# LordLiang/DrawingSpinUp

Hardware: AMD Instinct MI355X
Metric: drawings/sec end-to-end (512x512, 6 views, 24 frames) (higher is better)
Workload: dtype f16 (diffusion) / f16 table + f32 MLP (NSR) / f32 (stage-1 deformable convolutions, IS-Net, contour) / f32 with bf16 x 3 products (stage-2 convolutions; the reference: cuDNN TF32)

## Files before the change

### drawingspinup_amd/csrc/hashgrid_mfma.hip

```cpp
#include "hashgrid_dev.h"
#include "partial_reduce.h"
#include "tr_stage.h"

#include <type_traits>

using namespace dsu_hg;

namespace {

typedef float f32x16 __attribute__((ext_vector_type(16)));
typedef __bf16 bf16x8 __attribute__((ext_vector_type(8)));

__device__ __forceinline__ void softplus_inplace2(f32x16& acc, int r) {
  const f32x2 h = softplus100_pair(f32x2{acc[r], acc[r + 1]});
  acc[r] = h.x;
  acc[r + 1] = h.y;
}

__device__ __forceinline__ void bf16_split8(const float* x, bf16x8& hi, bf16x8& mid) {
#pragma unroll
  for (int i = 0; i < 8; ++i) {
    const __bf16 h = (__bf16)x[i];
    hi[i] = h;
    mid[i] = (__bf16)(x[i] - (float)h);
// ... 961 lines not shown
      const float dga = ax == 0 ? dg[0] : (ax == 1 ? dg[1] : dg[2]);
      dout0 = valid ? sgn * 0.5f * dga / eps + dl / eps2 : 0.0f;
    };
    if (e < 7) {
#pragma unroll
      for (int l = 0; l < ACT; ++l) vm_take(rw[l]);
      prep_unpack();
      prep_point(e);
      prep_request(e);
      prep_dout(e);
    }
#pragma unroll 1
    for (; e < 7; e += e_step) {
      gb1[0] += dout0;
      const float other0 = partner32(dout0, h);
      const float d0h0 = h == 0 ? dout0 : other0;
      const float d0h1 = h == 1 ? dout0 : other0;
      bf16x8 obh0, obm0, obh1, obm1;
      if constexpr (L0BF)
        pack_operands(in, std::integral_constant<int, (2 * KPA <= 16 ? 2 * KPA : 16)>{}, obh0, obm0, obh1, obm1);
#pragma unroll
      for (int half = 0; half < 2; ++half) {
        if (half == 1 && !live1) break;
        weights_per_use();
        const float d0 = half ? d0h1 : d0h0;
        f32x16 Hh[2];
        if constexpr (L0BF) l0_bf(half ? obh1 : obh0, half ? obm1 : obm0, Hh);
        else l0_half(in, half, Hh);
        softplus2(Hh);
#pragma unroll
        for (int T = 0; T < 2; ++T)
#pragma unroll
          for (int r = 0; r < 16; ++r) gw1c0[T][r] = fmaf(Hh[T][r], d0, gw1c0[T][r]);
        f32x16 din;
#pragma unroll
        for (int r = 0; r < 16; ++r) din[r] = 0.0f;
#pragma unroll
        for (int T = 0; T < 2; ++T) {
          float dpre[16];
#pragma unroll
          for (int q = 0; q < 4; ++q) {
            const float4 w = *reinterpret_cast<const float4*>(&lds[wo + PW_W1O0 + 32 * T + 8 * q + 4 * h]);
            dpre[4 * q + 0] = w.x * d0;
            dpre[4 * q + 1] = w.y * d0;
            dpre[4 * q + 2] = w.z * d0;
            dpre[4 * q + 3] = w.w * d0;
          }
          din_tile(T, dpre, Hh[T], din);
        }
        if (h == half) stage_in_T(in);
        __builtin_amdgcn_wave_barrier();
        gemm_T(gw0);
        __builtin_amdgcn_wave_barrier();
        store_din(e, din, wave_first + half * 32 + l31, r1);
      }
      const int en = e + e_step < 7 ? e + e_step : 6;
      handover();
      prep_unpack();
      prep_point(en);
      prep_request(en);
      prep_dout(en);
    }
#pragma unroll
    for (int T = 0; T < 2; ++T)
#pragma unroll
      for (int r = 0; r < 16; ++r) {
        float c0 = gw1c0[T][r];
#pragma unroll
        for (int off = 16; off > 0; off >>= 1) c0 += __shfl_xor(c0, off);
        if (l31 == gw1_col(0)) gw0[T][r] += c0;
      }
  }

  __syncthreads();
  float* red = lds;
  {
    float* rr = red + wave * PART_STRIDE;
#pragma unroll
    for (int T = 0; T < 2; ++T)
#pragma unroll
      for (int r = 0; r < 16; ++r) {
        const int feat = feat_of(T, r, h);
        const bool input = l31 < 2 * ACT || (l31 >= 2 * NL && l31 < 2 * NL + 4);
        rr[PART_GW0 + feat * 32 + l31] = input ? gw0[T][r] : 0.0f;
        const int o = l31 >= 2 * NL + 4 ? l31 - (2 * NL + 4) : (l31 >= 2 * ACT && l31 < 2 * ACT + NOUT - 8 ? l31 - 2 * ACT + 8 : -1);
        if (o >= 0) rr[PART_GW1 + feat * 32 + o] = gw0[T][r];
        if (l31 >= NOUT) rr[PART_GW1 + feat * 32 + l31] = 0.0f;
      }
#pragma unroll
    for (int o = 0; o < NOUT; ++o) gb1[o] += __shfl_xor(gb1[o], 32);
#pragma unroll
    for (int off = 16; off > 0; off >>= 1)
#pragma unroll
      for (int o = 0; o < NOUT; ++o) gb1[o] += __shfl_xor(gb1[o], off);
    if (lane == 0) {
#pragma unroll
      for (int o = 0; o < NOUT; ++o) rr[PART_GB1 + o] = gb1[o];
    }
  }
  __syncthreads();
  float* part = partials + (size_t)blockIdx.x * PART_STRIDE;
  for (int v = threadIdx.x; v < PART_GB1 + NOUT; v += blockDim.x)
    part[v] = (red[v] + red[PART_STRIDE + v]) + (red[2 * PART_STRIDE + v] + red[3 * PART_STRIDE + v]);
}

template <int NL, int ACT>
bool launch_bwd_pipe_one(uint32_t active, int blocks, hipStream_t s, const dsu_sdf_mlp& mlp,
                         const float* pts, int64_t n, float radius, float eps, float eps2,
                         const float* d_sdf, const float* d_grad, const float* d_feature,
                         const float* d_laplace, float* partials, const __half2* enc, float2* dinbuf,
                         const int32_t* perm) {
  if ((int)active != ACT) return false;
  sdf_fd_bwd_pipe_kernel<NL, ACT><<<dim3(blocks), dim3(256), 0, s>>>(
      mlp, pts, n, radius, eps, eps2, d_sdf, d_grad, d_feature, d_laplace, partials, enc, dinbuf, perm);
  return true;
}

template <int NL>
bool launch_bwd_pipe(uint32_t active, int blocks, hipStream_t s, const dsu_sdf_mlp& mlp,
                     const float* pts, int64_t n, float radius, float eps, float eps2,
                     const float* d_sdf, const float* d_grad, const float* d_feature,
                     const float* d_laplace, float* partials, const __half2* enc, float2* dinbuf,
                     const int32_t* perm) {
#define DSU_PIPE_TRY(A)                                                                          \
  if (launch_bwd_pipe_one<NL, A>(active, blocks, s, mlp, pts, n, radius, eps, eps2, d_sdf,       \
                                 d_grad, d_feature, d_laplace, partials, enc, dinbuf, perm))      \
    return true;
  DSU_PIPE_TRY(4) DSU_PIPE_TRY(5) DSU_PIPE_TRY(6) DSU_PIPE_TRY(7)
#undef DSU_PIPE_TRY
  return false;
}

constexpr int SC_MAXBLOCKS = 768;
constexpr int SC_THREADS = 256;
constexpr int SC_QCAP = 512;
constexpr int SC_LOG2 = 10;
constexpr int SC_SLOTS = 1 << SC_LOG2;
constexpr int SC_LDS_F = SC_SLOTS + 4 * SC_SLOTS + (SC_THREADS / 64) * 3 * SC_QCAP;
constexpr int SC_TILE_CAP = (SC_LDS_F * 4) / 16;
constexpr int SC_BBOX_OFF = SC_LDS_F;
constexpr int SC_LDS_TOTAL = SC_LDS_F + 16;
static_assert(SC_QCAP % 4 == 0 && SC_QCAP >= 512, "queue: one full evaluation of a wave must fit");

__device__ __forceinline__ uint32_t sc_slot(uint32_t entry) {
  return (entry * 2654435761u) >> (32 - SC_LOG2);
}
__device__ __forceinline__ void sc_commit_from(uint32_t* keys, unsigned long long* acc,
                                               float* __restrict__ gtable, uint32_t entry,
                                               uint32_t slot, float v0, float v1) {
#pragma unroll
  for (int probe = 1; probe < 3; ++probe) {
    slot = (slot + 1) & (SC_SLOTS - 1);
    const uint32_t old = atomicCAS(&keys[slot], GC_EMPTY, entry);
    if (old == GC_EMPTY || old == entry) {
      atomicAdd(&acc[2 * slot], gc_fix(v0));
      atomicAdd(&acc[2 * slot + 1], gc_fix(v1));
      return;
    }
  }
  unsafeAtomicAdd(gtable + (size_t)entry * 2, v0);
  unsafeAtomicAdd(gtable + (size_t)entry * 2 + 1, v1);
}

struct OwnReduce {
  const float* partials;
  int nblocks;
  float *g_w0, *g_b0, *g_w1, *g_b1;
};
constexpr int OWN_RED_BLOCKS = (PART_GB1 + NOUT + 63) / 64;

template <int NL>
__device__ __forceinline__ void reduce_own_block(const OwnReduce& o, int blk, float* red) {
  const int e = threadIdx.x & 63, g = threadIdx.x >> 6, ng = blockDim.x >> 6;
  const int v = blk * 64 + e;
  const bool in_range = v < PART_GB1 + NOUT;
  for (int sl = g; sl < 16; sl += ng) {
    float acc = 0.0f;
    if (in_range)
      for (int b = sl; b < o.nblocks; b += 16) acc += o.partials[(size_t)b * PART_STRIDE + v];
    red[sl * 64 + e] = acc;
  }
  __syncthreads();
  if (g != 0 || !in_range) return;
  float s = 0.0f;
#pragma unroll
  for (int k = 0; k < 16; ++k) s += red[k * 64 + e];
  if (v < PART_GW1) {
    const int feat = v >> 5, k = v & 31;
    if (k < MC<NL>::KIN) {
      const int c = ref_col<NL>(k);
      if (c >= 0) o.g_w0[feat * MC<NL>::DIN + c] += s;
      else o.g_b0[feat] += s;
    }
  } else if (v < PART_GB1) {
    const int feat = (v - PART_GW1) >> 5, oo = (v - PART_GW1) & 31;
    if (oo < NOUT) o.g_w1[oo * HID + feat] += s;
  } else {
    o.g_b1[v - PART_GB1] += s;
  }
}

template <int NL>
__global__ __launch_bounds__(SC_THREADS) void sdf_fd_scatter_kernel(
    GridMeta m, const float* __restrict__ pts, int64_t n, float radius, float eps, uint32_t active,
    const float2* __restrict__ dinbuf, float* __restrict__ gtable, int merge_levels,
    int centre_acc, int dense_levels, int* __restrict__ work_counter, OwnReduce own,
    dsu_partial_reduce extra) {
  extern __shared__ __attribute__((aligned(16))) float lds[];
  const int n_red_own = own.partials ? OWN_RED_BLOCKS : 0;
  const int n_red = n_red_own + (extra.partials ? dsu_red::blocks_of(extra) : 0);
  if ((int)blockIdx.x < n_red) {
    if ((int)blockIdx.x < n_red_own) reduce_own_block<NL>(own, blockIdx.x, lds);
    else dsu_red::reduce_block(extra, blockIdx.x - n_red_own, lds);
    return;
  }
  const int sc_block = (int)blockIdx.x - n_red, sc_grid = (int)gridDim.x - n_red;
  uint32_t* c_keys = reinterpret_cast<uint32_t*>(lds);
  unsigned long long* c_acc = reinterpret_cast<unsigned long long*>(lds + SC_SLOTS);
  const int lane = threadIdx.x & 63, wave = threadIdx.x >> 6;
  float* qbase = lds + 5 * SC_SLOTS + wave * 3 * SC_QCAP;
  uint32_t* q_ent = reinterpret_cast<uint32_t*>(qbase);
  float* q_v0 = qbase + SC_QCAP;
  float* q_v1 = qbase + 2 * SC_QCAP;
  unsigned long long* tile = reinterpret_cast<unsigned long long*>(lds);
  int* bbox = reinterpret_cast<int*>(lds + SC_BBOX_OFF);
  for (int t = threadIdx.x; t < SC_SLOTS; t += blockDim.x) {
    c_keys[t] = GC_EMPTY;
    c_acc[2 * t] = 0ull;
    c_acc[2 * t + 1] = 0ull;
  }
  if (threadIdx.x < 12) bbox[threadIdx.x] = (threadIdx.x % 6) < 3 ? 0x7fffffff : -0x7fffffff;
  int region = 0;
  __syncthreads();
  const int64_t n_chunks = (n + blockDim.x - 1) / blockDim.x;
  const int64_t n_items = n_chunks * (int64_t)active;
  int* next_slot = reinterpret_cast<int*>(lds + SC_BBOX_OFF) + 12;
  int64_t cur = sc_block, nxt = (int64_t)sc_block + sc_grid;
  float pn[3] = {0.f, 0.f, 0.f};
  float2 dnx[7];
#pragma unroll
  for (int e = 0; e < 7; ++e) dnx[e] = make_float2(0.f, 0.f);
  auto request = [&](int64_t item) {
    const int64_t chunk = item / (int64_t)active;
    const uint32_t lv = (uint32_t)(item - chunk * (int64_t)active);
    int64_t idx = chunk * blockDim.x + threadIdx.x;
    idx = idx < n ? idx : n - 1;
    pn[0] = pts[idx * 3]; pn[1] = pts[idx * 3 + 1]; pn[2] = pts[idx * 3 + 2];
#pragma unroll
    for (int e = 0; e < 7; ++e) dnx[e] = dinbuf[((size_t)e * active + lv) * n + idx];
  };
  if (cur < n_items) request(cur);
  int parity = 0;
  int qn = 0;
  auto drain = [&]() {
    __builtin_amdgcn_wave_barrier();
    for (int i0 = 0; i0 < qn; i0 += 64) {
      const int qi = i0 + lane;
      if (qi < qn) {
        const uint32_t ent = q_ent[qi];
        const float a0 = q_v0[qi], a1 = q_v1[qi];
        const uint32_t slot = sc_slot(ent);
        const uint32_t old = atomicCAS(&c_keys[slot], GC_EMPTY, ent);
        if (old == GC_EMPTY || old == ent) {
          atomicAdd(&c_acc[2 * slot], gc_fix(a0));
          atomicAdd(&c_acc[2 * slot + 1], gc_fix(a1));
        } else {
          sc_commit_from(c_keys, c_acc, gtable, ent, slot, a0, a1);
        }
      }
    }
    __builtin_amdgcn_wave_barrier();
    qn = 0;
  };
  auto flush_cache = [&]() {
    for (int t = threadIdx.x; t < SC_SLOTS; t += blockDim.x) {
      const uint32_t key = c_keys[t];
      if (key != GC_EMPTY) {
        unsafeAtomicAdd(gtable + (size_t)key * 2, gc_unfix(c_acc[2 * t]));
        unsafeAtomicAdd(gtable + (size_t)key * 2 + 1, gc_unfix(c_acc[2 * t + 1]));
        c_keys[t] = GC_EMPTY;
        c_acc[2 * t] = 0ull;
        c_acc[2 * t + 1] = 0ull;
      }
    }
  };

#pragma unroll 1
  while (cur < n_items) {
    {
      const int64_t chunk = cur / (int64_t)active;
      const int lev = (int)(cur - chunk * (int64_t)active);
      const float l_scale = m.scale[lev];
      const uint32_t l_off = m.off[lev], hsize = m.off[lev + 1] - m.off[lev];
      const uint32_t l_res = m.res[lev], l_hashed = m.hashed[lev];
      const int64_t i = chunk * blockDim.x + threadIdx.x;
      const bool valid = i < n;
      const float p[3] = {pn[0], pn[1], pn[2]};
      float2 dv[7];
#pragma unroll
      for (int e = 0; e < 7; ++e) {
        dv[e].x = valid ? dnx[e].x : 0.0f;
        dv[e].y = valid ? dnx[e].y : 0.0f;
      }
      if (nxt < n_items) request(nxt);
      if (threadIdx.x == 0) *next_slot = 2 * sc_grid + atomicAdd(work_counter, 1);
      const CellPos ccp = cell_of(l_scale, contract(p[0], radius), contract(p[1], radius),
                                  contract(p[2], radius));
      float2 D0 = dv[0], Da[3];
      uint32_t left = 0u;
      const bool inside = fabsf(p[0]) <= radius && fabsf(p[1]) <= radius && fabsf(p[2]) <= radius;
      int lo[3], hi[3];
#pragma unroll
      for (int a = 0; a < 3; ++a) {
        Da[a] = make_float2(0.f, 0.f);
        lo[a] = valid ? (int)ccp.c[a] : 0x7fffffff;
        hi[a] = valid ? (int)ccp.c[a] : -0x7fffffff;
      }
#pragma unroll
      for (int e = 1; e < 7; ++e) {
        const int ax = (e - 1) >> 1;
        const float off = ((e - 1) & 1) ? -eps : eps;
        const float qa = fminf(fmaxf(p[ax] + off, -radius), radius);
        const float posa = fmaf(l_scale, contract(qa, radius), 0.5f);
        const float fl = floorf(posa);
        const bool same = ((uint32_t)(int)fl == ccp.c[ax]) & (centre_acc != 0) & inside;
        const float delta = posa - ((float)(int)ccp.c[ax] + ccp.f[ax]);
        D0.x += same ? dv[e].x : 0.0f;
        D0.y += same ? dv[e].y : 0.0f;
        Da[ax].x += same ? dv[e].x * delta : 0.0f;
        Da[ax].y += same ? dv[e].y * delta : 0.0f;
        left |= (valid & !same) ? (1u << e) : 0u;
        if (valid & inside) {
          lo[ax] = min(lo[ax], (int)fl);
          hi[ax] = max(hi[ax], (int)fl);
        }
      }
      if (valid & !inside) {
#pragma unroll 1
        for (int e = 1; e < 7; ++e) {
          float q[3];
          fd_point(p, e, eps, radius, q);
          const CellPos cq = cell_of(l_scale, contract(q[0], radius), contract(q[1], radius),
                                     contract(q[2], radius));
#pragma unroll
          for (int a = 0; a < 3; ++a) {
            lo[a] = min(lo[a], (int)cq.c[a]);
            hi[a] = max(hi[a], (int)cq.c[a]);
          }
        }
      }
      bool dense = false;
      int x0 = 0, y0 = 0, z0 = 0, ddx = 1, ddxy = 1, vol = 0;
      int64_t after_next;
      {
        int* bb = bbox + 6 * parity;
#pragma unroll
        for (int a = 0; a < 3; ++a) {
#pragma unroll
          for (int off = 32; off > 0; off >>= 1) {
            lo[a] = min(lo[a], __shfl_xor(lo[a], off));
            hi[a] = max(hi[a], __shfl_xor(hi[a], off));
          }
        }
        if (lane == 0) {
#pragma unroll
          for (int a = 0; a < 3; ++a) {
            atomicMin(&bb[a], lo[a]);
            atomicMax(&bb[3 + a], hi[a]);
          }
        }
        __syncthreads();
        after_next = *next_slot;
        x0 = bb[0]; y0 = bb[1]; z0 = bb[2];
        const long long ex = (long long)bb[3] - x0 + 2, ey = (long long)bb[4] - y0 + 2,
                        ez = (long long)bb[5] - z0 + 2;
        if (dense_levels && bb[3] >= bb[0] && ex * ey * ez <= (long long)SC_TILE_CAP && ex < 4096 && ey < 4096) {
          dense = true;
          ddx = (int)ex; ddxy = (int)(ex * ey); vol = (int)(ex * ey * ez);
        }
        if (threadIdx.x < 6) bbox[6 * (parity ^ 1) + threadIdx.x] = threadIdx.x < 3 ? 0x7fffffff : -0x7fffffff;
        parity ^= 1;
      }
      if ((int)dense != region) {
        if (region == 0) {
          for (int t = threadIdx.x; t < SC_TILE_CAP * 2; t += blockDim.x) tile[t] = 0ull;
        } else {
          for (int t = threadIdx.x; t < SC_SLOTS; t += blockDim.x) {
            c_keys[t] = GC_EMPTY;
            c_acc[2 * t] = 0ull;
            c_acc[2 * t + 1] = 0ull;
          }
        }
        region = (int)dense;
        __syncthreads();
      }

#pragma unroll 1
      for (int e = 1; e < 8; ++e) {
        CellPos cp = ccp;
        float v[16];
        bool flush;
        if (e < 7) {
          flush = (left >> e) & 1u;
          if (__ballot(flush) == 0ull) continue;
          float2 d = dv[1];
#pragma unroll
          for (int k = 2; k < 7; ++k) {
            d.x = e == k ? dv[k].x : d.x;
            d.y = e == k ? dv[k].y : d.y;
          }
          float q[3];
          fd_point(p, e, eps, radius, q);
          cp = cell_of(l_scale, contract(q[0], radius), contract(q[1], radius), contract(q[2], radius));
#pragma unroll
          for (int c = 0; c < 8; ++c) {
            const float w = corner_weight(cp, c);
            v[2 * c] = w * d.x;
            v[2 * c + 1] = w * d.y;
          }
        } else {
          const float X[2] = {1.0f - cp.f[0], cp.f[0]}, Y[2] = {1.0f - cp.f[1], cp.f[1]},
                      Z[2] = {1.0f - cp.f[2], cp.f[2]};
#pragma unroll
          for (int c = 0; c < 8; ++c) {
            const int cx_ = c & 1, cy_ = (c >> 1) & 1, cz_ = (c >> 2) & 1;
            const float yz = Y[cy_] * Z[cz_], xz = X[cx_] * Z[cz_], xy = X[cx_] * Y[cy_];
            const float w = X[cx_] * yz;
            const float gx = cx_ ? yz : -yz, gy = cy_ ? xz : -xz, gz = cz_ ? xy : -xy;
            v[2 * c] = fmaf(D0.x, w, fmaf(Da[0].x, gx, fmaf(Da[1].x, gy, Da[2].x * gz)));
            v[2 * c + 1] = fmaf(D0.y, w, fmaf(Da[0].y, gx, fmaf(Da[1].y, gy, Da[2].y * gz)));
          }
          flush = valid;
        }
        const int key = flush ? (int)((cp.c[0] & 1023u) | ((cp.c[1] & 1023u) << 10) | ((cp.c[2] & 1023u) << 20))
                              : (0x40000000 | lane);
#pragma unroll
        for (int k = 0; k < 16; ++k) v[k] = flush ? v[k] : 0.0f;
        bool lead = flush;
        const int key_next = dpp_i<0x101>(key), key_prev = dpp_i<0x111>(key);
        const int l15 = lane & 15;
        const bool starts = ((l15 == 0) | (key_prev != key)) & flush;
        const int n_flush = __popcll(__ballot(flush)), n_start = __popcll(__ballot(starts));
        if (lev < merge_levels && 4 * n_start <= 3 * n_flush) {
          int ee = ((l15 == 15) | (key_next != key)) ? 1 : 0;
#define DSU_SEG_STEP(CTRL)                                              \
          {                                                             \
            const int eo = dpp_i<CTRL>(ee);                             \
            _Pragma("unroll") for (int k = 0; k < 16; ++k) {            \
              const float vo = dpp_f<CTRL>(v[k]);                       \
              v[k] += ee ? 0.0f : vo;                                   \
            }                                                           \
            ee |= eo;                                                   \
          }
          DSU_SEG_STEP(0x101) DSU_SEG_STEP(0x102) DSU_SEG_STEP(0x104) DSU_SEG_STEP(0x108)
#undef DSU_SEG_STEP
          lead = starts;
        }
        if (dense) {
          if (lead) {
            const int base = ((int)cp.c[0] - x0) + ((int)cp.c[1] - y0) * ddx + ((int)cp.c[2] - z0) * ddxy;
#pragma unroll
            for (int c = 0; c < 8; ++c) {
              const int t = base + (c & 1) + ((c >> 1) & 1) * ddx + ((c >> 2) & 1) * ddxy;
              atomicAdd(&tile[2 * t], gc_fix(v[2 * c]));
              atomicAdd(&tile[2 * t + 1], gc_fix(v[2 * c + 1]));
            }
          }
          continue;
        }
        const unsigned long long bal = __ballot(lead);
        if (lead) {
          const int pos = qn + 8 * __popcll(bal & ((1ull << lane) - 1ull));
          uint32_t ent[8];
#pragma unroll
          for (int c = 0; c < 8; ++c)
            ent[c] = l_off + grid_index(l_hashed, hsize, l_res, cp.c[0] + (c & 1),
                                        cp.c[1] + ((c >> 1) & 1), cp.c[2] + ((c >> 2) & 1));
#pragma unroll
          for (int q4 = 0; q4 < 2; ++q4) {
            *reinterpret_cast<uint4*>(&q_ent[pos + 4 * q4]) =
                make_uint4(ent[4 * q4], ent[4 * q4 + 1], ent[4 * q4 + 2], ent[4 * q4 + 3]);
            *reinterpret_cast<float4*>(&q_v0[pos + 4 * q4]) =
                make_float4(v[8 * q4], v[8 * q4 + 2], v[8 * q4 + 4], v[8 * q4 + 6]);
            *reinterpret_cast<float4*>(&q_v1[pos + 4 * q4]) =
                make_float4(v[8 * q4 + 1], v[8 * q4 + 3], v[8 * q4 + 5], v[8 * q4 + 7]);
          }
        }
        qn += 8 * __popcll(bal);
        if (qn + 512 > SC_QCAP) drain();
      }
      if (!dense) drain();
      __syncthreads();
      if (dense) {
        for (int t = threadIdx.x; t < vol; t += blockDim.x) {
          const unsigned long long a0 = tile[2 * t], a1 = tile[2 * t + 1];
          if (a0 | a1) {
            const int z = t / ddxy, rr = t - z * ddxy;
            const int y = rr / ddx, x = rr - y * ddx;
            const uint32_t g = l_off + grid_index(l_hashed, hsize, l_res, (uint32_t)(x0 + x),
                                                  (uint32_t)(y0 + y), (uint32_t)(z0 + z));
            unsafeAtomicAdd(gtable + (size_t)g * 2, gc_unfix(a0));
            unsafeAtomicAdd(gtable + (size_t)g * 2 + 1, gc_unfix(a1));
            tile[2 * t] = 0ull;
            tile[2 * t + 1] = 0ull;
          }
        }
      } else {
        flush_cache();
      }
      cur = nxt;
      nxt = after_next;
    }
  }
}

constexpr int BWD_MFMA_MAX_BLOCKS = 512;

}

#define DSU_DISPATCH_NL(nl, ...)                       \
  switch (nl) {                                        \
    case 10: { constexpr int NL = 10; __VA_ARGS__ } break; \
    case 12: { constexpr int NL = 12; __VA_ARGS__ } break; \
    default: return DSU_EUNSUP;                        \
  }

extern "C" {

int64_t dsu_sdf_fd_enc_cache_bytes(int64_t n, uint32_t active_levels) {
  if (n < 0 || active_levels > DSU_MAX_LEVELS) return DSU_EINVAL;
  return (int64_t)7 * n * active_levels * 4;
}

int64_t dsu_sdf_fd_bwd_workspace_bytes(const dsu_hashgrid_cfg* cfg, int64_t n) {
  if (!cfg || n < 0) return DSU_EINVAL;
  if (cfg->n_levels != 10 && cfg->n_levels != 12) return DSU_EUNSUP;
  const int blocks = dsu_capped_blocks(n, 256, BWD_MFMA_MAX_BLOCKS);
  return (int64_t)blocks * PART_STRIDE * sizeof(float) +
         (int64_t)7 * n * cfg->n_levels * (int64_t)sizeof(float2) + 256;
}

int dsu_sdf_fd_bwd_sorted(const dsu_hashgrid_cfg* cfg, const void* table_f16, const dsu_sdf_mlp* mlp,
                   const float* pts, const int32_t* perm, int64_t n, float radius, float eps,
                   uint32_t active_levels, const float* d_sdf, const float* d_grad,
                   const float* d_feature, const float* d_laplace, float* grad_table,
                   float* g_w0, float* g_b0, float* g_w1, float* g_b1, void* workspace,
                   int64_t workspace_bytes, const void* enc_cache, void* stream) {
  return dsu_sdf_fd_bwd_sorted_fold(cfg, table_f16, mlp, pts, perm, n, radius, eps, active_levels,
                                    d_sdf, d_grad, d_feature, d_laplace, grad_table, g_w0, g_b0, g_w1,
                                    g_b1, workspace, workspace_bytes, enc_cache, nullptr, nullptr,
                                    stream);
}

int dsu_sdf_fd_bwd_sorted_fold(const dsu_hashgrid_cfg* cfg, const void* table_f16,
                               const dsu_sdf_mlp* mlp, const float* pts, const int32_t* perm,
                               int64_t n, float radius, float eps, uint32_t active_levels,
                               const float* d_sdf, const float* d_grad, const float* d_feature,
                               const float* d_laplace, float* grad_table, float* g_w0, float* g_b0,
                               float* g_w1, float* g_b1, void* workspace, int64_t workspace_bytes,
                               const void* enc_cache, void* mid_event,
                               const dsu_partial_reduce* extra, void* stream) {
  if (extra && (!extra->partials || !extra->map || !extra->base || extra->nblocks < 0 ||
                extra->n <= 0 || extra->stride < extra->n))
    return DSU_EINVAL;
  if (extra && n == 0) return DSU_EUNSUP;
  if (!cfg || !table_f16 || !mlp || (!pts && n) || n < 0) return DSU_EINVAL;
  if (!mlp->w0 || !mlp->b0 || !mlp->w1 || !mlp->b1) return DSU_EINVAL;
  if (!grad_table || !g_w0 || !g_b0 || !g_w1 || !g_b1) return DSU_EINVAL;
  if (active_levels > cfg->n_levels || !(eps > 0.0f)) return DSU_EINVAL;
  GridMeta m;
  int rc = make_meta(cfg, &m);
  if (rc) return rc;
  for (uint32_t l = 0; l < active_levels; ++l)
    if (m.res[l] + 1u > 1024u) return DSU_EUNSUP;
  if (n == 0) return DSU_OK;
  const int64_t need = dsu_sdf_fd_bwd_workspace_bytes(cfg, n);
  if (need < 0) return (int)need;
  if (!workspace || workspace_bytes < need) return DSU_EINVAL;
  hipStream_t s = (hipStream_t)stream;
  const float eps2 = (float)((double)eps * (double)eps);
  const bool two_per_cu = cfg->n_levels == 10 && enc_cache && active_levels >= 4 && active_levels <= 6;
  const int blocks = dsu_onewave_blocks(n, 256, BWD_MFMA_MAX_BLOCKS, two_per_cu ? 2 : 1);
  const size_t shm1 = (size_t)K1_LDS_F * sizeof(float);
  const size_t shm2 = (size_t)SC_LDS_TOTAL * sizeof(float);
  float2* dinbuf = reinterpret_cast<float2*>((char*)workspace +
                                             (size_t)blocks * PART_STRIDE * sizeof(float));
  int sblocks = dsu_capped_blocks(n, SC_THREADS, SC_MAXBLOCKS);
  if (dsu_scatter_grid_cap_value > 0 && sblocks > dsu_scatter_grid_cap_value) sblocks = dsu_scatter_grid_cap_value;
  DSU_DISPATCH_NL(cfg->n_levels, {
    auto k1 = enc_cache ? sdf_fd_bwd_mfma_kernel<NL, true> : sdf_fd_bwd_mfma_kernel<NL, false>;
    auto k2 = sdf_fd_scatter_kernel<NL>;
    DSU_ENSURE_DYN_LDS((sdf_fd_bwd_mfma_kernel<NL, true>), shm1);
    DSU_ENSURE_DYN_LDS((sdf_fd_bwd_mfma_kernel<NL, false>), shm1);
    DSU_ENSURE_DYN_LDS(k2, shm2);
    bool piped = false;
    if constexpr (NL == 10) {
      if (enc_cache)
        piped = launch_bwd_pipe<NL>(active_levels, blocks, s, *mlp, pts, n, radius, eps, eps2,
                                    d_sdf, d_grad, d_feature, d_laplace, (float*)workspace,
                                    (const __half2*)enc_cache, dinbuf, perm);
    }
    if (!piped)
      k1<<<dim3(blocks), dim3(256), shm1, s>>>(
          (const __half2*)table_f16, m, *mlp, pts, n, radius, eps, eps2, active_levels, d_sdf,
          d_grad, d_feature, d_laplace, (float*)workspace, (const __half2*)enc_cache, dinbuf, perm);
    if (mid_event && hipEventRecord((hipEvent_t)mid_event, s) != hipSuccess) return DSU_ELAUNCH;
    int* work_counter = reinterpret_cast<int*>(dinbuf + (size_t)7 * (size_t)n * cfg->n_levels);
    const OwnReduce own{(const float*)workspace, blocks, g_w0, g_b0, g_w1, g_b1};
    dsu_partial_reduce ext{};
    if (extra) ext = *extra;
    const int n_red = OWN_RED_BLOCKS + (extra ? dsu_red::blocks_of(ext) : 0);
    k2<<<dim3(n_red + sblocks), dim3(SC_THREADS), shm2, s>>>(m, pts, n, radius, eps, active_levels,
                                                            dinbuf, grad_table,  64,
                                                             1,  1,
                                                            work_counter, own, ext);
  });
  DSU_CHECK_LAUNCH();
  return DSU_OK;
}

}
```

Measured before the change: 0.3613.

## Fold face-adjacent finite-difference samples into centre-cell scatter in hashgrid backward

```diff
diff --git a/drawingspinup_amd/csrc/hashgrid_mfma.hip b/drawingspinup_amd/csrc/hashgrid_mfma.hip
--- a/drawingspinup_amd/csrc/hashgrid_mfma.hip
+++ b/drawingspinup_amd/csrc/hashgrid_mfma.hip
@@ -1287,26 +1287,34 @@
         dv[e].x = valid ? dnx[e].x : 0.0f;
         dv[e].y = valid ? dnx[e].y : 0.0f;
       }
+      float cc[9];
+#pragma unroll
+      for (int a = 0; a < 3; ++a) cc[a] = contract(p[a], radius);
+#pragma unroll
+      for (int e = 1; e < 7; ++e) {
+        const float off = ((e - 1) & 1) ? -eps : eps;
+        cc[2 + e] = contract(fminf(fmaxf(p[(e - 1) >> 1] + off, -radius), radius), radius);
+      }
       if (nxt < n_items) request(nxt);
       if (threadIdx.x == 0) *next_slot = 2 * sc_grid + atomicAdd(work_counter, 1);
-      const CellPos ccp = cell_of(l_scale, contract(p[0], radius), contract(p[1], radius),
-                                  contract(p[2], radius));
+      const CellPos ccp = cell_of(l_scale, cc[0], cc[1], cc[2]);
       float2 D0 = dv[0], Da[3];
-      uint32_t left = 0u;
+      float2 Sf[3][2];
+      uint32_t left = 0u, face = 0u;
       const bool inside = fabsf(p[0]) <= radius && fabsf(p[1]) <= radius && fabsf(p[2]) <= radius;
       int lo[3], hi[3];
 #pragma unroll
       for (int a = 0; a < 3; ++a) {
         Da[a] = make_float2(0.f, 0.f);
+        Sf[a][0] = make_float2(0.f, 0.f);
+        Sf[a][1] = make_float2(0.f, 0.f);
         lo[a] = valid ? (int)ccp.c[a] : 0x7fffffff;
         hi[a] = valid ? (int)ccp.c[a] : -0x7fffffff;
       }
 #pragma unroll
       for (int e = 1; e < 7; ++e) {
         const int ax = (e - 1) >> 1;
-        const float off = ((e - 1) & 1) ? -eps : eps;
-        const float qa = fminf(fmaxf(p[ax] + off, -radius), radius);
-        const float posa = fmaf(l_scale, contract(qa, radius), 0.5f);
+        const float posa = fmaf(l_scale, cc[2 + e], 0.5f);
         const float fl = floorf(posa);
         const bool same = ((uint32_t)(int)fl == ccp.c[ax]) & (centre_acc != 0) & inside;
         const float delta = posa - ((float)(int)ccp.c[ax] + ccp.f[ax]);
@@ -1314,7 +1322,15 @@
         D0.y += same ? dv[e].y : 0.0f;
         Da[ax].x += same ? dv[e].x * delta : 0.0f;
         Da[ax].y += same ? dv[e].y * delta : 0.0f;
-        left |= (valid & !same) ? (1u << e) : 0u;
+        const int dc = (int)fl - (int)ccp.c[ax];
+        const bool fnb = valid & inside & (centre_acc != 0) & ((dc == 1) | (dc == -1));
+        const float fr = posa - fl, ws = dc > 0 ? 1.0f - fr : fr;
+        Sf[ax][1].x += (fnb & (dc > 0)) ? dv[e].x * ws : 0.0f;
+        Sf[ax][1].y += (fnb & (dc > 0)) ? dv[e].y * ws : 0.0f;
+        Sf[ax][0].x += (fnb & (dc < 0)) ? dv[e].x * ws : 0.0f;
+        Sf[ax][0].y += (fnb & (dc < 0)) ? dv[e].y * ws : 0.0f;
+        face |= fnb ? (1u << e) : 0u;
+        left |= (valid & !same & !fnb) ? (1u << e) : 0u;
         if (valid & inside) {
           lo[ax] = min(lo[ax], (int)fl);
           hi[ax] = max(hi[ax], (int)fl);
@@ -1380,47 +1396,17 @@
         __syncthreads();
       }
 
-#pragma unroll 1
-      for (int e = 1; e < 8; ++e) {
-        CellPos cp = ccp;
-        float v[16];
-        bool flush;
-        if (e < 7) {
-          flush = (left >> e) & 1u;
-          if (__ballot(flush) == 0ull) continue;
-          float2 d = dv[1];
-#pragma unroll
-          for (int k = 2; k < 7; ++k) {
-            d.x = e == k ? dv[k].x : d.x;
-            d.y = e == k ? dv[k].y : d.y;
-          }
-          float q[3];
-          fd_point(p, e, eps, radius, q);
-          cp = cell_of(l_scale, contract(q[0], radius), contract(q[1], radius), contract(q[2], radius));
-#pragma unroll
-          for (int c = 0; c < 8; ++c) {
-            const float w = corner_weight(cp, c);
-            v[2 * c] = w * d.x;
-            v[2 * c + 1] = w * d.y;
-          }
-        } else {
-          const float X[2] = {1.0f - cp.f[0], cp.f[0]}, Y[2] = {1.0f - cp.f[1], cp.f[1]},
-                      Z[2] = {1.0f - cp.f[2], cp.f[2]};
-#pragma unroll
-          for (int c = 0; c < 8; ++c) {
-            const int cx_ = c & 1, cy_ = (c >> 1) & 1, cz_ = (c >> 2) & 1;
-            const float yz = Y[cy_] * Z[cz_], xz = X[cx_] * Z[cz_], xy = X[cx_] * Y[cy_];
-            const float w = X[cx_] * yz;
-            const float gx = cx_ ? yz : -yz, gy = cy_ ? xz : -xz, gz = cz_ ? xy : -xy;
-            v[2 * c] = fmaf(D0.x, w, fmaf(Da[0].x, gx, fmaf(Da[1].x, gy, Da[2].x * gz)));
-            v[2 * c + 1] = fmaf(D0.y, w, fmaf(Da[0].y, gx, fmaf(Da[1].y, gy, Da[2].y * gz)));
-          }
-          flush = valid;
-        }
-        const int key = flush ? (int)((cp.c[0] & 1023u) | ((cp.c[1] & 1023u) << 10) | ((cp.c[2] & 1023u) << 20))
+      auto emit = [&](auto nc_tag, const uint32_t (&cell)[3], const uint32_t (&org)[3], int ua, int va,
+                      float* v, bool flush) {
+        constexpr int NC = decltype(nc_tag)::value;
+        auto off = [&](int k, int a) -> int {
+          if (NC == 8) return (k >> a) & 1;
+          return (a == ua ? (k & 1) : 0) + (a == va ? (k >> 1) : 0);
+        };
+        const int key = flush ? (int)((cell[0] & 1023u) | ((cell[1] & 1023u) << 10) | ((cell[2] & 1023u) << 20))
                               : (0x40000000 | lane);
 #pragma unroll
-        for (int k = 0; k < 16; ++k) v[k] = flush ? v[k] : 0.0f;
+        for (int k = 0; k < 2 * NC; ++k) v[k] = flush ? v[k] : 0.0f;
         bool lead = flush;
         const int key_next = dpp_i<0x101>(key), key_prev = dpp_i<0x111>(key);
         const int l15 = lane & 15;
@@ -1431,7 +1417,7 @@
 #define DSU_SEG_STEP(CTRL)                                              \
           {                                                             \
             const int eo = dpp_i<CTRL>(ee);                             \
-            _Pragma("unroll") for (int k = 0; k < 16; ++k) {            \
+            _Pragma("unroll") for (int k = 0; k < 2 * NC; ++k) {        \
               const float vo = dpp_f<CTRL>(v[k]);                       \
               v[k] += ee ? 0.0f : vo;                                   \
             }                                                           \
@@ -1443,26 +1429,26 @@
         }
         if (dense) {
           if (lead) {
-            const int base = ((int)cp.c[0] - x0) + ((int)cp.c[1] - y0) * ddx + ((int)cp.c[2] - z0) * ddxy;
-#pragma unroll
-            for (int c = 0; c < 8; ++c) {
-              const int t = base + (c & 1) + ((c >> 1) & 1) * ddx + ((c >> 2) & 1) * ddxy;
+            const int base = ((int)org[0] - x0) + ((int)org[1] - y0) * ddx + ((int)org[2] - z0) * ddxy;
+#pragma unroll
+            for (int c = 0; c < NC; ++c) {
+              const int t = base + off(c, 0) + off(c, 1) * ddx + off(c, 2) * ddxy;
               atomicAdd(&tile[2 * t], gc_fix(v[2 * c]));
               atomicAdd(&tile[2 * t + 1], gc_fix(v[2 * c + 1]));
             }
           }
-          continue;
+          return;
         }
         const unsigned long long bal = __ballot(lead);
         if (lead) {
-          const int pos = qn + 8 * __popcll(bal & ((1ull << lane) - 1ull));
-          uint32_t ent[8];
-#pragma unroll
-          for (int c = 0; c < 8; ++c)
-            ent[c] = l_off + grid_index(l_hashed, hsize, l_res, cp.c[0] + (c & 1),
-                                        cp.c[1] + ((c >> 1) & 1), cp.c[2] + ((c >> 2) & 1));
-#pragma unroll
-          for (int q4 = 0; q4 < 2; ++q4) {
+          const int pos = qn + NC * __popcll(bal & ((1ull << lane) - 1ull));
+          uint32_t ent[NC];
+#pragma unroll
+          for (int c = 0; c < NC; ++c)
+            ent[c] = l_off + grid_index(l_hashed, hsize, l_res, org[0] + off(c, 0), org[1] + off(c, 1),
+                                        org[2] + off(c, 2));
+#pragma unroll
+          for (int q4 = 0; q4 < NC / 4; ++q4) {
             *reinterpret_cast<uint4*>(&q_ent[pos + 4 * q4]) =
                 make_uint4(ent[4 * q4], ent[4 * q4 + 1], ent[4 * q4 + 2], ent[4 * q4 + 3]);
             *reinterpret_cast<float4*>(&q_v0[pos + 4 * q4]) =
@@ -1471,8 +1457,82 @@
                 make_float4(v[8 * q4 + 1], v[8 * q4 + 3], v[8 * q4 + 5], v[8 * q4 + 7]);
           }
         }
-        qn += 8 * __popcll(bal);
+        qn += NC * __popcll(bal);
         if (qn + 512 > SC_QCAP) drain();
+      };
+#pragma unroll 1
+      for (int e = 1; e < 8; ++e) {
+        CellPos cp = ccp;
+        float v[16];
+        bool flush;
+        if (e < 7) {
+          const bool fb = (face >> e) & 1u;
+          flush = (left >> e) & 1u;
+          const bool any_face = __ballot(fb) != 0ull, any_cell = __ballot(flush) != 0ull;
+          if (!any_face && !any_cell) continue;
+          const int ax = (e - 1) >> 1;
+          float2 d = dv[1];
+          float ce = cc[3];
+#pragma unroll
+          for (int k = 2; k < 7; ++k) {
+            d.x = e == k ? dv[k].x : d.x;
+            d.y = e == k ? dv[k].y : d.y;
+            ce = e == k ? cc[2 + k] : ce;
+          }
+          const float posa = fmaf(l_scale, ce, 0.5f), fl = floorf(posa), fr = posa - fl;
+          if (any_face) {
+            const int ua = ax == 0 ? 1 : 0, va = ax == 2 ? 1 : 2;
+            const float fu = ax == 0 ? ccp.f[1] : ccp.f[0], fv = ax == 2 ? ccp.f[1] : ccp.f[2];
+            const uint32_t ca = ax == 0 ? ccp.c[0] : (ax == 1 ? ccp.c[1] : ccp.c[2]);
+            const bool up = (int)fl > (int)ca;
+            const float wn = up ? fr : 1.0f - fr;
+            const float dx = wn * d.x, dy = wn * d.y;
+            const float U[2] = {1.0f - fu, fu}, V[2] = {1.0f - fv, fv};
+            uint32_t cell[3], org[3];
+#pragma unroll
+            for (int a = 0; a < 3; ++a) {
+              cell[a] = a == ax ? (uint32_t)(int)fl : ccp.c[a];
+              org[a] = a == ax ? (uint32_t)((int)fl + (up ? 1 : 0)) : ccp.c[a];
+            }
+            float vf[8];
+#pragma unroll
+            for (int k = 0; k < 4; ++k) {
+              const float w = U[k & 1] * V[k >> 1];
+              vf[2 * k] = dx * w;
+              vf[2 * k + 1] = dy * w;
+            }
+            emit(std::integral_constant<int, 4>{}, cell, org, ua, va, vf, fb);
+          }
+          if (!any_cell) continue;
+          float q[3];
+          fd_point(p, e, eps, radius, q);
+          cp = cell_of(l_scale, contract(q[0], radius), contract(q[1], radius), contract(q[2], radius));
+#pragma unroll
+          for (int c = 0; c < 8; ++c) {
+            const float w = corner_weight(cp, c);
+            v[2 * c] = w * d.x;
+            v[2 * c + 1] = w * d.y;
+          }
+        } else {
+          const float X[2] = {1.0f - cp.f[0], cp.f[0]}, Y[2] = {1.0f - cp.f[1], cp.f[1]},
+                      Z[2] = {1.0f - cp.f[2], cp.f[2]};
+          float2 A[3][2];
+#pragma unroll
+          for (int a = 0; a < 3; ++a) {
+            A[a][0] = make_float2(Sf[a][0].x - Da[a].x, Sf[a][0].y - Da[a].y);
+            A[a][1] = make_float2(Sf[a][1].x + Da[a].x, Sf[a][1].y + Da[a].y);
+          }
+#pragma unroll
+          for (int c = 0; c < 8; ++c) {
+            const int cx_ = c & 1, cy_ = (c >> 1) & 1, cz_ = (c >> 2) & 1;
+            const float yz = Y[cy_] * Z[cz_], xz = X[cx_] * Z[cz_], xy = X[cx_] * Y[cy_];
+            const float w = X[cx_] * yz;
+            v[2 * c] = fmaf(D0.x, w, fmaf(A[0][cx_].x, yz, fmaf(A[1][cy_].x, xz, A[2][cz_].x * xy)));
+            v[2 * c + 1] = fmaf(D0.y, w, fmaf(A[0][cx_].y, yz, fmaf(A[1][cy_].y, xz, A[2][cz_].y * xy)));
+          }
+          flush = valid;
+        }
+        emit(std::integral_constant<int, 8>{}, cp.c, cp.c, 0, 0, v, flush);
       }
       if (!dense) drain();
       __syncthreads();
```

Result: no change. 0.3594 (-0.5%).
